# Happy-ZZX/PL-VIWO

Hardware: AMD Instinct MI355X
Metric: frames/sec (track+EKF update), 752x480 mono, 250 pts+80 lines; ATE vs CPU ref (higher is better)
Workload: dtype f64

## Files before the change

### pl-viwo_amd/csrc/dense_kernels.hip

```cpp
#include "mfma_tile.hpp"
#include "update_kernels.hpp"
#include "wave_ops.hpp"

namespace plv {


static inline int cdiv(int a, int b) { return (a + b - 1) / b; }

__global__ void __launch_bounds__(256) gram_direct_kernel(const double *__restrict__ A, int lda, int nc, const int *__restrict__ acc_rows, int F,
                                                          int mp_max, double *__restrict__ G, const int *__restrict__ skip,
                                                          double *__restrict__ Gs, double *__restrict__ gv) {
  if (skip && *skip == 0) return;
  __shared__ double part[3][256];
  const int nt = (nc + 15) >> 4;
  int rem = blockIdx.x, ti = 0;
  while (rem >= nt - ti) {
    rem -= nt - ti;
    ++ti;
  }
  const int tj = ti + rem;
  const int wave = threadIdx.x >> 6, lane = threadIdx.x & 63, li = lane & 15;
  const double *ai = A + (size_t)min(ti * 16 + li, nc - 1) * lda;
  const double *aj = A + (size_t)min(tj * 16 + li, nc - 1) * lda;
  d4 acc = {0, 0, 0, 0};
// ... 96 lines not shown
    for (int i = threadIdx.x; i < mirror2_words; i += blockDim.x) mirror2_dst[i] = mirror2_src[i];
  if (!(skipped || capped || *flag != 0)) {
    for (int idx = blockIdx.x * blockDim.x + threadIdx.x; idx < n * n; idx += gridDim.x * blockDim.x) {
      int j = idx / n, i = idx - j * n;
      if (i <= j) {
        const double u = P[(size_t)j * ldp + i];
        if (save) save[(size_t)j * n + i] = u, save[(size_t)i * n + j] = P[(size_t)i * ldp + j];
        double v = u - dC[(size_t)j * ldc + i];
        P[(size_t)j * ldp + i] = v;
        P[(size_t)i * ldp + j] = v;
      }
    }
  }
}

bool ekf_fast_fits(int r) { return r <= 192; }
static int launch_ekf_commit(plv_ctx *ctx, double *d_P, int n, int ldp, const double *dC, double *d_dx, int *d_flag, const void *mirror_src,
                             void *mirror_dst, size_t mirror_bytes);

int launch_ekf_fast(plv_ctx *ctx, double *d_P, int n, int ldp, const double *d_H, int r, int k, int ldh, const int *d_cols,
                    const double *d_res, const double *d_Rdiag, double *d_dx, int *d_flag, bool gathered, const void *mirror_src,
                    void *mirror_dst, size_t mirror_bytes) {
  int rc;
  const int ldm = r, ldw = r;
  if ((rc = ctx->d_Mt.reserve((size_t)r * (n + 1 + k) * 8)) || (rc = ctx->d_S.reserve((size_t)r * r * 8 * 2)) ||
      (rc = ctx->d_W.reserve((size_t)r * (n + 1) * 8)) || (rc = ctx->d_y.reserve((size_t)n * n * 8)))
    return rc;
  double *Mt = ctx->d_Mt.as<double>(), *S = ctx->d_S.as<double>(), *W = ctx->d_W.as<double>(), *dC = ctx->d_y.as<double>();
  launch_ekf_ms(ctx, d_P, n, ldp, d_H, r, k, ldh, d_cols, d_Rdiag, Mt, ldm, S, gathered, d_flag);
  if ((rc = launch_bchol_ekf(ctx, S, r, r, Mt, ldm, n, d_res, W, ldw, d_flag))) return rc;
  {
    ProfScope ps(ctx->prof, "ekf_dc_kernel", ctx->stream);
    int tn = cdiv(n + 1, 16);
    int waves = tn * (tn + 1) / 2;
    hipLaunchKernelGGL(ekf_dc_kernel, dim3(cdiv(waves, 4)), dim3(256), 0, ctx->stream, W, ldw, r, n, dC, n, d_dx, d_P, ldp, d_flag, ctx->skip_word,
                       (const double *)nullptr, (const double *)nullptr, (const double *)nullptr, (const int *)nullptr);
  }
  return launch_ekf_commit(ctx, d_P, n, ldp, dC, d_dx, d_flag, mirror_src, mirror_dst, mirror_bytes);
}

static int launch_ekf_commit(plv_ctx *ctx, double *d_P, int n, int ldp, const double *dC, double *d_dx, int *d_flag, const void *mirror_src,
                             void *mirror_dst, size_t mirror_bytes) {
  {
    ProfScope ps(ctx->prof, "ekf_commit_kernel", ctx->stream);
    hipLaunchKernelGGL(ekf_commit_kernel, dim3(std::min(64, cdiv(n * n, 256))), dim3(256), 0, ctx->stream, d_P, ldp, n, dC, n,
                       d_flag, (const unsigned *)mirror_src, (unsigned *)mirror_dst, (int)(mirror_bytes / 4), ctx->skip_word, d_dx,
                       (const unsigned *)(mirror_dst ? ctx->mirror2_src : nullptr), (unsigned *)(mirror_dst ? ctx->mirror2_dst : nullptr),
                       (int)((ctx->mirror2_bytes + 3) / 4), mirror_dst ? ctx->applied_word : nullptr,
                       mirror_dst ? ctx->cap_words : nullptr, ctx->cap, ctx->cov_save, ctx->cov_save_word, ctx->cov_save_seq);
    if (mirror_dst && ctx->applied_word) ctx->applied_used = true;
    if (mirror_dst && ctx->mirror2_dst) ctx->mirror2_taken = true;
  }
  PLV_HIP_CHECK(hipGetLastError());
// ... 113 lines not shown
                        void *mirror_dst, size_t mirror_bytes) {
  int rc;
  if ((rc = ctx->d_Mt.reserve((size_t)k * 8)) || (rc = ctx->d_S.reserve((size_t)k * k * 8)) || (rc = ctx->d_W.reserve((size_t)k * (n + 1) * 8)) ||
      (rc = ctx->d_y.reserve((size_t)n * n * 8)))
    return rc;
  double *cv = ctx->d_Mt.as<double>(), *B = ctx->d_S.as<double>(), *V = ctx->d_W.as<double>(), *dC = ctx->d_y.as<double>();
  const double *Gs = ctx->d_Gs.as<double>(), *gv = Gs + (size_t)k * k;
  if ((rc = ctx->d_C1.reserve(((size_t)n * n + n) * 8)) || (rc = ctx->d_Y0.reserve((size_t)k * (n + 1) * 8)) || (rc = ctx->d_GP.reserve((size_t)k * n * 8)))
    return rc;
  double *Y0 = ctx->d_Y0.as<double>(), *C1 = ctx->d_C1.as<double>(), *d0 = C1 + (size_t)n * n, *GP = ctx->d_GP.as<double>();
  const int *use_m = ctx->d_prior_near.as<int>();
  if (plv::knob(plv::PLV_KNOB_FORCE_FACTOR_FORM)) {
    static const int one[2] = {1, 0};
    PLV_HIP_CHECK(hipMemcpyAsync(ctx->d_prior_near.p, one, 8, hipMemcpyHostToDevice, ctx->stream));
  }
  launch_whiten_b(ctx, ctx->d_Lt.as<double>(), k, Gs, gv, cv, B, d_flag, d_P, ldp, n, d_cols, Y0, GP, d0, use_m);
  const WhitenC1Args wc{d_P, ldp, d_cols, GP, C1, Y0, use_m};
  if ((rc = launch_bchol_ekf(ctx, B, k, k, ctx->d_W0.as<double>(), k, n, cv, V, k, d_flag, &wc))) return rc;
  {
    ProfScope ps(ctx->prof, "ekf_dc_kernel", ctx->stream);
    const int tn = cdiv(n + 1, 16), waves = tn * (tn + 1) / 2;
    hipLaunchKernelGGL(ekf_dc_kernel, dim3(cdiv(waves, 4)), dim3(256), 0, ctx->stream, V, k, k, n, dC, n, d_dx, d_P, ldp, d_flag, ctx->skip_word,
                       ctx->d_dW.as<double>(), C1, d0, use_m);
  }
  return launch_ekf_commit(ctx, d_P, n, ldp, dC, d_dx, d_flag, mirror_src, mirror_dst, mirror_bytes);
}

}
```

### pl-viwo_amd/csrc/line_api.hip

```cpp
#include <algorithm>
#include <chrono>
#include <cmath>
#include <cstring>
#include <atomic>
#include <condition_variable>
#include <functional>
#include <memory>
#include <map>
#include <mutex>
#include <thread>
#include <unordered_map>
#include <vector>

#include "line_host.hpp"
#include "cam_models.hpp"
#include "line_kernels.hpp"
#include "update_state.hpp"
#include "plv_internal.hpp"
#include "camera_tracks.hpp"
#include "update_tail.hpp"

using namespace plv;
using namespace plv::linehost;

// ... 62 lines not shown
  struct WalkInfo {
    int mode = 0, n_components = 0, longest_component = 0, n_chains = 0, fell_back = 0;
  } winfo;
  bool chains_valid = false;
  std::vector<FldChain> last_chains;
  int last_pts_extent = 0;
  DevBuf comps, recs, recs_sorted;
  bool prefetch = false;
  std::unordered_map<uint64_t, LineTrack> db;
  DevBuf half, map, work, pts, chains, counts, segs, seg_count, uv_in, uv_out;
  DevBuf lab, lab_cnt, lab_roots;
  hipStream_t ccl_stream = nullptr;
  hipEvent_t canny_done = nullptr, labels_ready = nullptr;
  PinBuf pin;
  hipEvent_t edges_ready = nullptr;
  std::vector<uint64_t> dec_ids;
  std::vector<double> dec_vals;
  const uint8_t *early_raw = nullptr;
  const unsigned *early_hist = nullptr;
  int early_w = 0, early_h = 0;
  int pending_which = -1, pending_fed = -1;
  bool defer_finish = false;
  std::function<void()> deferred;
  std::atomic<int> defer_state{0};
  struct TriState {
    bool valid = false;
    plv_state_view view;
    std::vector<double> clone_time, clone_R, clone_p;
    std::vector<int> clone_id;
  } tri_state;
// ... 65 lines not shown
      F.pool_on = false;
      plv::frame_mark("@ (worker) line feed + pool done");
      plv::counters().w_feed_ns += (unsigned long long)std::chrono::duration_cast<std::chrono::nanoseconds>(std::chrono::steady_clock::now() - Fs).count();
      {
        std::lock_guard<std::mutex> lk(T->jm);
        F.rc = rc;
        T->feed_state = 2;
      }
      T->jcv.notify_all();
      continue;
    }
    const bool timing = plv::knob(plv::PLV_KNOB_LINE_TIMING);
    auto W0 = std::chrono::steady_clock::now();
    (void)hipSetDevice(T->job.device);
    int rc = PLV_OK;
    if (plv::event_sync(T->edges_ready) != hipSuccess) rc = PLV_E_DEVICE;
    if (rc == PLV_OK && T->job.hlab && plv::event_sync(T->labels_ready) != hipSuccess) rc = PLV_E_DEVICE;
    auto W1 = std::chrono::steady_clock::now();
    if (rc == PLV_OK) rc = host_extract(&T->host, T->job, timing);
    {
      auto ns = [](auto a, auto b) { return (unsigned long long)std::chrono::duration_cast<std::chrono::nanoseconds>(b - a).count(); };
      plv::counters().w_wake_ns += ns(T->job_posted, W0);
      plv::counters().w_maps_ns += ns(W0, W1);
      plv::counters().w_extract_ns += ns(W1, std::chrono::steady_clock::now());
    }
    if (plv::host_phases().on)
      plv::host_phases().add("line worker: detect job, post to done", std::chrono::duration<double, std::micro>(std::chrono::steady_clock::now() - T->job_posted).count());
    plv::frame_mark("@ (worker) line detection done");
    if (timing) {
      auto W2 = std::chrono::steady_clock::now();
      auto us = [](auto a, auto b) { return std::chrono::duration<double, std::micro>(b - a).count(); };
// ... 119 lines not shown
    b.lab_cnt = T->lab_cnt.as<int>();
    b.lab_roots = T->lab_roots.as<int>();
    b.comps = T->comps.as<FldComp>();
    b.recs = T->recs.as<FldRec>();
    b.recs_sorted = T->recs_sorted.as<FldRec>();
    b.walk_info = T->counts.as<int>() + 4;
  }
  if (!prelaunched) TRY(launch_line_edges(ctx, d_img, W, H, fp, b, ctx->stream, early ? T->early_hist : nullptr));
  if (with_labels && !T->ccl_stream) {
    PLV_HIP_CHECK(hipStreamCreateWithFlags(&T->ccl_stream, hipStreamNonBlocking));
    PLV_HIP_CHECK(hipEventCreateWithFlags(&T->canny_done, hipEventDisableTiming));
    PLV_HIP_CHECK(hipEventCreateWithFlags(&T->labels_ready, hipEventDisableTiming));
  }
  if (with_labels) PLV_HIP_CHECK(hipEventRecord(T->canny_done, ctx->stream));
  if (launch_only && !T->edges_ready) PLV_HIP_CHECK(hipEventCreateWithFlags(&T->edges_ready, hipEventDisableTiming));
  if (launch_only && maps_to_host) PLV_HIP_CHECK(hipEventRecord(T->edges_ready, ctx->stream));
  if (early && ctx->after_edges) TRY(ctx->after_edges(ctx->after_edges_arg));
  if (with_labels) {
    PLV_HIP_CHECK(hipStreamWaitEvent(T->ccl_stream, T->canny_done, 0));
    TRY(launch_line_labels(ctx, w, h, b, T->ccl_stream, fp.length_threshold));
    PLV_HIP_CHECK(hipEventRecord(T->labels_ready, T->ccl_stream));
  }
  const float thr2 = ctx->cfg.line_min_length_px * ctx->cfg.line_min_length_px;
  auto emit = [&](const float4 &sg) {
    const float x1 = sg.x * 2, y1 = sg.y * 2, x2 = sg.z * 2, y2 = sg.w * 2;
    const float l2 = (x2 - x1) * (x2 - x1) + (y2 - y1) * (y2 - y1);
    if (!(l2 > thr2)) return;
    lines.insert(lines.end(), {x1, y1, x2, y2});
  };
  lines.clear();
  if (!T->walk_on_device) {
// ... 1012 lines not shown
```

### pl-viwo_amd/csrc/plv_api.hip

```cpp
#include <algorithm>
#include <cstdarg>
#include <dlfcn.h>
#include <cmath>
#include <mutex>

#include "plv_ctx.hpp"
#include "update_kernels.hpp"
#include "update_state.hpp"

namespace plv {

static thread_local char g_err[512] = "";
void set_last_error(const char *fmt, ...) {
  va_list ap;
  va_start(ap, fmt);
  vsnprintf(g_err, sizeof(g_err), fmt, ap);
  va_end(ap);
}

double chi2_quantile(int dof, double p);

Roctx::Roctx() {
  if (!getenv("PLV_ROCTX")) return;
  for (const char *name : {"librocprofiler-sdk-roctx.so", "libroctx64.so"}) {
// ... 225 lines not shown
    g_states.push_back({ctx, us});
  }
  *out = ctx;
  return PLV_OK;
}

void plv_ctx_destroy(plv_ctx *ctx) {
  if (!ctx) return;
  (void)hipSetDevice(ctx->device);
  (void)plv::stream_sync(ctx->stream);
  plv_tracker_destroy(ctx);
  plv_line_tracker_destroy(ctx);
  plv_frontend_destroy(ctx);
  ctx->prof.destroy();
  plv::DevBuf *bufs[] = {&ctx->d_P, &ctx->d_P2, &ctx->d_H, &ctx->d_res, &ctx->d_cols, &ctx->d_Rdiag, &ctx->d_dx, &ctx->d_flag,
                         &ctx->d_Mt, &ctx->d_S, &ctx->d_W, &ctx->d_y, &ctx->d_fHf, &ctx->d_fHx, &ctx->d_fres,
                         &ctx->d_frows, &ctx->d_chi2, &ctx->d_acc, &ctx->d_stack, &ctx->d_stack_l, &ctx->d_stack2, &ctx->d_Pc, &ctx->d_Ps,
                         &ctx->d_inv, &ctx->d_T, &ctx->d_Lt, &ctx->d_W0, &ctx->d_dW, &ctx->d_Gs};
  for (auto *b : bufs) b->release();
  if (ctx->aux_stream) {
    (void)plv::stream_sync(ctx->aux_stream);
    (void)hipStreamDestroy(ctx->aux_stream);
  }
  if (ctx->aux_fork) (void)hipEventDestroy(ctx->aux_fork);
  if (ctx->aux_join) (void)hipEventDestroy(ctx->aux_join);
  ctx->h_pin.release();
  ctx->h_pin_flow.release();
  ctx->h_pin_l.release();
  plv_ctx_update_state *us = nullptr;
  {
    std::lock_guard<std::mutex> lk(g_state_mtx);
// ... 520 lines not shown
  const size_t rb = result_rows_off(n, F) + (size_t)F * 4;
  plv::PinBuf &hpin = ctx->res_pin(fdim);
  TRY(hpin.reserve(rb));
  struct SkipGuard {
    plv_ctx *c;
    ~SkipGuard() { c->skip_word = nullptr; }
  } skip_guard{ctx};
  const bool whiten = whitened_route(us, Mtot, k);
  bool aux_open = prior_was_pending;
  auto aux_join = [&]() -> int {
    if (!aux_open) return PLV_OK;
    aux_open = false;
    PLV_HIP_CHECK(hipStreamWaitEvent(ctx->stream, ctx->aux_join, 0));
    return PLV_OK;
  };
  const bool probing = ctx->probe && !us->graph_mode;
  auto start_prior = [&]() -> int {
    TRY(aux_join());
    TRY(prior_mark(ctx, true));
    TRY(prior_start(ctx, us->bcols_of(fdim).as<int>(), k));
    aux_open = true;
    return PLV_OK;
  };
  auto enqueue = [&]() -> int {
  if (whiten && !prefetched && !probing) TRY(start_prior());
  if (!projected) {
    TRY(launch_nullspace(ctx, F, fdim, k, ld, us->brows.as<int>(), wHf, wHx, wres, ctx->d_P.as<double>(), n, n, us->bcols_of(fdim).as<int>()));
  } else if (!gathers_valid) {
    TRY(launch_gather_cov(ctx, ctx->d_P.as<double>(), n, n, us->bcols_of(fdim).as<int>(), k));
  }
  Chi2Args a{};
// ... 19 lines not shown
    ctx->dec_F_l = F;
  }
  a.stack = ctx->stack_of(fdim).as<double>();
  a.lds = Mtot;
  a.mp_max = mp_max;
  a.chi2_mult = chi2_mult;
  a.res_norm_gate = res_norm_gate;
  a.q95 = us->q95.as<double>();
  a.q95_n = Q95_N;
  a.min_rows = fdim == 3 ? 4 : 5;
  a.accepted = d_acc;
  a.acc_rows = d_acc_rows;
  a.n_acc = d_flag + 1;
  a.stack_accepted_only = (Mtot > k && k <= 192 && whiten) ? 1 : 0;
  ctx->skip_word = (Mtot > k ? k <= 192 : ekf_fast_fits(Mtot)) ? d_flag + 1 : nullptr;
  const bool probe = ctx->probe && !us->graph_mode;
  if (probe) {
    char *hb = hpin.as<char>();
    a.h_accepted = (unsigned char *)(hb + (size_t)n * 8 + 16);
    a.h_acc_rows = (int *)(hb + result_rows_off(n, F));
    a.probe_src = (const unsigned char *)ctx->probe_src;
    a.probe_dst = (unsigned char *)ctx->probe_dst;
    a.probe_stride_a = ctx->probe_stride_a, a.probe_off_b = ctx->probe_off_b, a.probe_stride_b = ctx->probe_stride_b;
  }
  const bool gated = ctx->gate_stage_taken && projected && ctx->gate_stage.stack == a.stack && ctx->gate_stage.lds == a.lds &&
                     ctx->gate_stage.accepted == a.accepted && ctx->gate_stage.stack_accepted_only == a.stack_accepted_only;
  if (ctx->gate_stage_taken && !gated) {
    set_last_error("plv_msckf_update_resident: the batch was gated inside its Jacobian launch for other buffers than this update's");
    return PLV_E_BADARG;
  }
  if (gated) {
// ... 11 lines not shown
    if (ctx->probe_hook) ctx->probe_hook(ctx->probe_hook_arg);
    TRY(sync(ctx));
    const unsigned char *hacc = (const unsigned char *)(hpin.as<char>() + (size_t)n * 8 + 16);
    int any = 0;
    for (int f = 0; f < F; ++f) any |= hacc[f];
    if (!any) {
      memset(hpin.p, 0, (size_t)n * 8 + 16);
      ctx->probe_done = true;
      return aux_join();
    }
    const int *hrows = (const int *)(hpin.as<char>() + result_rows_off(n, F));
    int m_acc = 0;
    for (int f = 0; f < F; ++f) m_acc += std::max(hrows[f], 0);
    if (whiten && m_acc > 0 && m_acc <= k && ekf_fast_fits(m_acc) && !plv::knob(plv::PLV_KNOB_FORCE_FACTOR_FORM)) {
      TRY(ctx->d_stackc.reserve((size_t)m_acc * nc * 8));
      TRY(launch_stack_compact(ctx, ctx->stack_of(fdim).as<double>(), Mtot, nc, d_acc_rows, F, mp_max, ctx->d_stackc.as<double>(), m_acc, true));
      TRY(aux_join());
      const double *Hc = ctx->d_stackc.as<double>();
      TRY(launch_ekf_fast(ctx, ctx->d_P.as<double>(), n, n, Hc, m_acc, k, m_acc, us->bcols_of(fdim).as<int>(), Hc + (size_t)k * m_acc, nullptr, d_dx, d_flag,
                          gathers_valid, resbuf.p, hpin.p, (rb + 3) & ~(size_t)3));
      us->last_route = 0;
      return PLV_OK;
    }
    if (whiten && !prefetched) TRY(start_prior());
  }

  const double *dH, *dr;
  int r, ldh;
  if (whiten) {
    TRY(launch_gram_information(ctx, ctx->stack_of(fdim).as<double>(), Mtot, nc, d_acc_rows, F, mp_max));
// ... 219 lines not shown
```

### pl-viwo_amd/csrc/plv_ctx.hpp

```cpp
#pragma once
#include <hip/hip_runtime.h>
#include <sys/resource.h>

#include "gate_stage.hpp"
#include <cstdint>
#include <cstdio>
#include <execinfo.h>
#include <cstring>
#include <algorithm>
#include <atomic>
#include <chrono>
#include <cstdlib>
#include <mutex>
#include <string>
#include <unordered_map>
#include <vector>

#include "../../include/plviwo.h"

namespace plv {

void set_last_error(const char *fmt, ...);

#define PLV_HIP_CHECK(expr)                                                              \
// ... 33 lines not shown
  counters().copy_bytes += bytes;
  return hipMemcpyAsync(dst, src, bytes, kind, s);
}

enum : unsigned { PLV_KNOB_PRIOR_LATE = 2u, PLV_KNOB_GATE_SEPARATE = 1024u, PLV_KNOB_NO_CHAIN = 2048u, PLV_KNOB_CHAIN_ALWAYS = 4096u,
                  PLV_KNOB_FORCE_FACTOR_FORM = 8192u,
                  PLV_KNOB_HOST_TIMING = 1u << 14,
                  PLV_KNOB_LINE_TIMING = 1u << 15,
                  PLV_KNOB_UPDATE_TIMING = 1u << 16,
                  PLV_KNOB_KERNEL_STAMPS = 1u << 17,
                  PLV_KNOB_CHAIN_EVENTS = 1u << 18,
                  PLV_KNOB_ALLOC_DEBUG = 1u << 19,
                  PLV_KNOB_HOST_FAULTS = 1u << 20,
                  PLV_KNOB_NO_SPECULATION = 1u << 24,
                  PLV_KNOB_HELPER_NAPS = 1u << 28,
                  PLV_KNOB_TSQR_TREE = 1u << 29 };
inline std::atomic<unsigned> &knobs() {
  static std::atomic<unsigned> k{getenv("PLV_DEBUG_KNOBS") ? (unsigned)strtoul(getenv("PLV_DEBUG_KNOBS"), nullptr, 0) : 0u};
  return k;
}
inline bool knob(unsigned bit) { return (knobs().load(std::memory_order_relaxed) & bit) != 0; }
inline bool alloc_debug() { return knob(PLV_KNOB_ALLOC_DEBUG); }

struct HostPhases {
  struct Rec {
    const char *label;
    double us = 0;
    long n = 0;
    float last[64] = {};
    void put(double v) {
      last[n & 63] = (float)v;
// ... 302 lines not shown

struct plv_ctx {
  plv_config cfg;
  int cam_model = 0;
  int device = 0;
  hipStream_t stream = nullptr;
  plv::Profiler prof;

  int cov_n = 0;
  unsigned long long gather_stamp = 1;
  unsigned long long cov_host_synced = 0;
  plv::DevBuf d_P;
  plv::DevBuf d_P2;
  plv::DevBuf d_H, d_res, d_cols, d_Rdiag, d_dx, d_flag;
  plv::DevBuf d_Mt, d_S, d_W, d_y;
  plv::DevBuf d_Pc, d_Ps, d_inv, d_T;
  plv::DevBuf d_fHf, d_fHx, d_fres, d_frows, d_chi2, d_acc;
  void (*edges_hook)(plv_ctx *, const uint8_t *d_raw, int W, int H, const unsigned *d_hist) = nullptr;
  bool edges_hook_fired = false;
  int (*after_edges)(void *) = nullptr;
  void *after_edges_arg = nullptr;
  bool decision_trace = false;
  plv::DevBuf d_tri_dbg, d_gate_dec, d_gate_dec_l;
  int dec_F_l = 0;
  int dec_F = 0;
  bool dec_gate = false;
  plv::DevBuf d_stack, d_stack2;
  plv::DevBuf d_stack_l;
  plv::DevBuf &stack_of(int fdim) { return fdim == 6 ? d_stack_l : d_stack; }
  plv::DevBuf d_Lt, d_W0, d_dW, d_Gs, d_GP, d_Y0, d_C1, d_stackc;
// ... 49 lines not shown
```

### pl-viwo_amd/csrc/update_kernels.hip

```cpp
#include <algorithm>

#include "plv_ctx.hpp"
#include "blocked_chol.hpp"
#include "mfma_tile.hpp"
#include "nullspace_core.hpp"
#include "update_kernels.hpp"

namespace plv {

template <class FA, class FB>
__device__ __forceinline__ d4 mfma_tile_f64(FA a, FB b, int K, d4 acc) {
  const int lane = threadIdx.x & 63;
  const int ij = lane & 15, kq = lane >> 4;
  int k0 = 0;
  for (; k0 + 16 <= K; k0 += 16) {
    double av[4], bv[4];
#pragma unroll
    for (int u = 0; u < 4; ++u) {
      av[u] = a(ij, k0 + 4 * u + kq);
      bv[u] = b(k0 + 4 * u + kq, ij);
    }
#pragma unroll
    for (int u = 0; u < 4; ++u) acc = __builtin_amdgcn_mfma_f64_16x16x4f64(av[u], bv[u], acc, 0, 0, 0);
  }
// ... 576 lines not shown
  const double *P;
  int ldp, n;
  const int *cols;
  const double *g;
  double *Y0;
  double *GP;
  double *d0;
  const int *use_m;
  int first;
};

__global__ void __launch_bounds__(512) ekf_ms_kernel(const double *__restrict__ H, int ldh, int r, int k, const double *__restrict__ Pc,
                                                     int ldp, int n, const double *__restrict__ Ps, double *__restrict__ Mt, int ldm,
                                                     const double *__restrict__ Rdiag, double *__restrict__ S, int lds_,
                                                     int mt_blocks, int *__restrict__ flag, const int *__restrict__ skip, int h_upper,
                                                     WhitenPanels wp) {
  __shared__ double strip[192 * 17];
  if (flag && blockIdx.x == 0 && threadIdx.x == 0) {
    flag[0] = 0;
  }
  if (skip && *skip == 0) return;
  const int wave = threadIdx.x >> 6, lane = threadIdx.x & 63, li = lane & 15, nw = blockDim.x >> 6;
  if ((int)blockIdx.x < mt_blocks) {
    const int tr_n = (r + 15) >> 4, tn_n = (n + 15) >> 4;
    const int tile = blockIdx.x * nw + wave;
    if (tile >= tr_n * tn_n) return;
    const int tr = tile / tn_n, tn = tile - tr * tn_n;
    d4 acc = {0, 0, 0, 0};
    const int k0 = h_upper ? min(tr * 16, k) : 0;
    const double *Hr = H + min(tr * 16 + li, r - 1) + (size_t)k0 * ldh;
    const double *Pq = Pc + min(tn * 16 + li, n - 1) + (size_t)k0 * ldp;
    auto fa = [&](int, int kk) { return Hr[(size_t)kk * ldh]; };
    auto fb = [&](int kk, int) { return Pq[(size_t)kk * ldp]; };
    acc = mfma_tile_f64_pipe<16>(fa, fb, k - k0, acc);
#pragma unroll
    for (int q = 0; q < 4; ++q) {
      const int i = tr * 16 + (lane >> 4) + 4 * q, j = tn * 16 + li;
      if (i < r && j < n) Mt[(size_t)j * ldm + i] = acc[q];
    }
    return;
  }
  const int kt = (k + 15) >> 4, tr_n = (r + 15) >> 4;
  if (wp.first >= 0 && (int)blockIdx.x >= wp.first) {
    __shared__ int scols[192];
    if ((wp.use_m[0] | wp.use_m[1]) == 0) return;
// ... 28 lines not shown
      const double *sp = strip + k0 * 17;
      auto fa = [&](int, int kk) { return Hr[(size_t)kk * ldh]; };
      auto fb = [&](int kk, int) { return sp[kk * 17 + li]; };
      acc = mfma_tile_f64_pipe<16>(fa, fb, k - k0, acc);
#pragma unroll
      for (int q = 0; q < 4; ++q) {
        const int c = tj * 16 + (lane >> 4) + 4 * q;
        if (c < k && b0 + li < wp.n) wp.Y0[(size_t)(b0 + li) * k + c] = acc[q];
      }
    }
    return;
  }
  const int ti = blockIdx.x - mt_blocks;
  {
    const int k0 = h_upper ? min(ti * 16, k) : 0;
    const double *Hr = H + min(ti * 16 + li, r - 1) + (size_t)k0 * ldh;
    for (int tj = wave; tj < kt; tj += nw) {
      d4 acc = {0, 0, 0, 0};
      const double *Pq = Ps + min(tj * 16 + li, k - 1) + (size_t)k0 * k;
      auto fa = [&](int, int kk) { return Hr[(size_t)kk * ldh]; };
      auto fb = [&](int kk, int) { return Pq[(size_t)kk * k]; };
      acc = mfma_tile_f64_pipe<16>(fa, fb, k - k0, acc);
#pragma unroll
      for (int q = 0; q < 4; ++q) {
        const int j = tj * 16 + li;
        if (j < k) strip[j * 17 + (lane >> 4) + 4 * q] = acc[q];
      }
    }
  }
  __syncthreads();
  for (int tj = ti + wave; tj < tr_n; tj += nw) {
    d4 acc = {0, 0, 0, 0};
    const int k0 = h_upper ? min(tj * 16, k) : 0;
    const double *Hc = H + min(tj * 16 + li, r - 1) + (size_t)k0 * ldh;
    const double *sp = strip + k0 * 17;
    auto fa = [&](int, int kk) { return sp[kk * 17 + li]; };
    auto fb = [&](int kk, int) { return Hc[(size_t)kk * ldh]; };
    acc = mfma_tile_f64_pipe<16>(fa, fb, k - k0, acc);
#pragma unroll
    for (int q = 0; q < 4; ++q) {
      const int i = ti * 16 + (lane >> 4) + 4 * q, j = tj * 16 + li;
      if (i < r && j < r) S[(size_t)j * lds_ + i] = acc[q] + (i == j ? (Rdiag ? Rdiag[i] : 1.0) : 0.0);
    }
  }
}

__global__ void __launch_bounds__(1024) ekf_chol_kernel(const double *__restrict__ S, int lds_, int r, double *__restrict__ L,
                                                        int ldl, int *__restrict__ flag) {
  extern __shared__ double smem[];
// ... 242 lines not shown
      *result = dst;
      *ld_out = ldo;
      return PLV_OK;
    }
    rows = W * nc;
    src_ld = ldo;
    double *t = src;
    src = dst;
    dst = t;
    size_t tc = cap_src;
    cap_src = cap_dst;
    cap_dst = tc;
  }
}

void launch_ekf_ms(plv_ctx *ctx, const double *d_P, int n, int ldp, const double *d_H, int r, int k, int ldh,
                   const int *d_cols, const double *d_Rdiag, double *Mt, int ldm, double *S, bool gathered, int *d_flag) {
  if (!gathered) (void)launch_gather_cov(ctx, d_P, n, ldp, d_cols, k);
  ProfScope ps(ctx->prof, "ekf_ms_kernel", ctx->stream);
  const int mt_blocks = cdiv(cdiv(r, 16) * cdiv(n, 16), 4);
  if (k > 192) {
    hipLaunchKernelGGL(ekf_mt_kernel, dim3(mt_blocks), dim3(256), 0, ctx->stream, d_H, ldh, r, k, ctx->d_inv.as<int>(),
                       ctx->d_Pc.as<double>(), n, n, Mt, ldm, d_flag, ctx->skip_word);
    hipLaunchKernelGGL(ekf_s_kernel, dim3(cdiv(cdiv(r, 16) * cdiv(r, 16), 4)), dim3(256), 0, ctx->stream, Mt + (size_t)(n + 1) * ldm, ldm,
                       d_H, ldh, r, k, d_cols, d_Rdiag, S, r, ctx->skip_word);
    return;
  }
  hipLaunchKernelGGL(ekf_ms_kernel, dim3(mt_blocks + cdiv(r, 16)), dim3(256), 0, ctx->stream, d_H, ldh, r, k, ctx->d_Pc.as<double>(), n, n,
                     ctx->d_Ps.as<double>(), Mt, ldm, d_Rdiag, S, r, mt_blocks, d_flag, ctx->skip_word, 0, WhitenPanels{nullptr, 0, 0, nullptr, nullptr, nullptr, nullptr, nullptr, nullptr, -1});
}

void launch_whiten_b(plv_ctx *ctx, const double *Lt, int k, const double *Gs, const double *gv, double *cv, double *B, int *d_flag,
                     const double *d_P, int ldp, int n, const int *d_cols, double *Y0, double *GP, double *d0, const int *use_m) {
  ProfScope ps(ctx->prof, "ekf_ms_kernel", ctx->stream);
  const int mt_blocks = cdiv(cdiv(k, 16), 8), first = mt_blocks + cdiv(k, 16);
  hipLaunchKernelGGL(ekf_ms_kernel, dim3(first + cdiv(n, 16)), dim3(512), 0, ctx->stream, Lt, k, k, k, gv, 1, 1, Gs, cv, k,
                     (const double *)nullptr, B, k, mt_blocks, d_flag, ctx->skip_word, 1, WhitenPanels{d_P, ldp, n, d_cols, gv, Y0, GP, d0, use_m, first});
}

int launch_ekf(plv_ctx *ctx, double *d_P, int n, int ldp, const double *d_H, int r, int k, int ldh, const int *d_cols,
               const double *d_res, const double *d_Rdiag, double *d_dx, int *d_flag, bool gathered) {
  int rc;
  const int ldm = r, ldw = r;
  if ((rc = ctx->d_Mt.reserve((size_t)r * (n + 1 + k) * 8)) || (rc = ctx->d_S.reserve((size_t)r * r * 8 * 2)) ||
      (rc = ctx->d_W.reserve((size_t)r * (n + 1) * 8)))
    return rc;
  double *Mt = ctx->d_Mt.as<double>(), *S = ctx->d_S.as<double>(), *L = S + (size_t)r * r, *W = ctx->d_W.as<double>();
  size_t shm = (size_t)r * (r | 1) * sizeof(double);
  if (shm > 160 * 1024) {
    set_last_error("ekf: r=%d exceeds the LDS-resident Cholesky capacity", r);
    return PLV_E_CAPACITY;
  }
// ... 25 lines not shown
```

### pl-viwo_amd/csrc/update_kernels.hpp

```cpp
#pragma once
#include "plv_ctx.hpp"

namespace plv {

struct Chi2Args {
  const double *P;
  int ldp;
  int k, ld, fdim_off;
  const int *rows;
  const double *Hx, *res;
  const int *cols;
  double sigma2;
  double *chi2;
  double *dec;
  double *stack;
  int lds, mp_max;
  double chi2_mult, res_norm_gate;
  const double *q95;
  int q95_n;
  int min_rows;
  unsigned char *accepted;
  int *acc_rows;
  int *n_acc;
  int stack_accepted_only;
// ... 7 lines not shown
  int probe_stride_a, probe_off_b, probe_stride_b;
};

int launch_nullspace(plv_ctx *ctx, int F, int fdim, int k, int ld, const int *d_rows, double *d_Hf, double *d_Hx,
                     double *d_res, const double *d_P = nullptr, int n = 0, int ldp = 0, const int *d_cols = nullptr,
                     int shift = -1 );
struct GatherArgs;
int gather_args(plv_ctx *ctx, const double *d_P, int n, int ldp, const int *d_cols, int k, GatherArgs &g);
int launch_gather_cov(plv_ctx *ctx, const double *d_P, int n, int ldp, const int *d_cols, int k);
int launch_chi2(plv_ctx *ctx, int F, const Chi2Args &a, int max_mp);
int launch_tsqr(plv_ctx *ctx, double *d_A, int lda, int m, int nc, double *d_tmp, size_t tmp_elems, double **result,
                int *ld_out, const int *m_dev = nullptr);
int launch_ekf(plv_ctx *ctx, double *d_P, int n, int ldp, const double *d_H, int r, int k, int ldh, const int *d_cols,
               const double *d_res, const double *d_Rdiag, double *d_dx, int *d_flag, bool gathered = false);

void launch_ekf_ms(plv_ctx *ctx, const double *d_P, int n, int ldp, const double *d_H, int r, int k, int ldh,
                   const int *d_cols, const double *d_Rdiag, double *Mt, int ldm, double *S, bool gathered = false,
                   int *d_flag = nullptr);
bool ekf_fast_fits(int r);
int launch_ekf_fast(plv_ctx *ctx, double *d_P, int n, int ldp, const double *d_H, int r, int k, int ldh, const int *d_cols,
                    const double *d_res, const double *d_Rdiag, double *d_dx, int *d_flag, bool gathered = false, const void *mirror_src = nullptr,
                    void *mirror_dst = nullptr, size_t mirror_bytes = 0);

void launch_whiten_b(plv_ctx *ctx, const double *Lt, int k, const double *Gs, const double *gv, double *cv, double *B, int *d_flag,
                     const double *d_P, int ldp, int n, const int *d_cols, double *Y0, double *GP, double *d0, const int *use_m);
int launch_stack_compact(plv_ctx *ctx, const double *d_A, int lda, int nc, const int *d_acc_rows, int F, int mp_max, double *d_dst, int ldd, bool exact_rows = false,
                         int *d_total_out = nullptr );
int launch_cov_restore(plv_ctx *ctx, double *d_P, int n, const double *save, const unsigned *save_word, unsigned seq);
int launch_stack_zero_rejected(plv_ctx *ctx, double *d_A, int lda, int nc, const int *d_acc_rows, int F, int mp_max);
int launch_prior_factor(plv_ctx *ctx, hipStream_t st, const double *d_P, int n, int ldp, const int *d_cols, int k);
int launch_gram_information(plv_ctx *ctx, const double *d_A, int lda, int nc, const int *d_acc_rows, int F, int mp_max);
int launch_ekf_whitened(plv_ctx *ctx, double *d_P, int n, int ldp, int k, const int *d_cols, double *d_dx, int *d_flag, const void *mirror_src, void *mirror_dst,
                        size_t mirror_bytes);
int launch_bchol_prior(plv_ctx *ctx, hipStream_t st, const double *d_P, int ldp, int n, const int *d_cols, int k, double *d_Lt, int ldl,
                       double *d_W0, int ldw, int *d_n_near);

int launch_cov_init_invertible(plv_ctx *ctx, const double *d_P, int n, const int *d_cols, int k, const double *d_Hx, const double *d_Hf,
                               const double *d_res, int ld, double *d_Pn, double *d_out, int *d_flag);

struct WhitenC1Args {
// ... 13 lines not shown
```

Measured before the change: 2001.

## Fuse EKF covariance-delta and commit into one kernel, read accepted rows in place

Adds a single-launch ekf_dc_commit kernel. Each block computes a tile of the covariance downdate and checks the diagonal for negativity using P's diagonal, which the ms kernel snapshots. It also writes dx, the mirror copies and P in place, replacing the separate dc and commit kernels and the dC scratch round-trip. The ms kernel can now read accepted measurement rows through a row map, so the stack-compaction launch is skipped on the whitened fast path. Line extraction waits on the canny event instead of a separate edges event. Together these cut launch count and memory traffic on the update tail, at the cost of a much more complex kernel and more blocks being launched.

```diff
diff --git a/pl-viwo_amd/csrc/dense_kernels.hip b/pl-viwo_amd/csrc/dense_kernels.hip
--- a/pl-viwo_amd/csrc/dense_kernels.hip
+++ b/pl-viwo_amd/csrc/dense_kernels.hip
@@ -134,29 +134,180 @@
   }
 }
 
+template <int NW, int CH>
+__global__ void __launch_bounds__(64 * NW) ekf_dc_commit_kernel(const double *__restrict__ W, int ldw, int r, int n, double *__restrict__ dx,
+                                                            double *__restrict__ P, int ldp, const double *__restrict__ pdiag,
+                                                            int *__restrict__ flag, const int *__restrict__ skip,
+                                                            const double *__restrict__ dW, const double *__restrict__ C1,
+                                                            const double *__restrict__ d0, const int *__restrict__ use_m,
+                                                            const unsigned *__restrict__ mirror_src, unsigned *__restrict__ mirror_dst,
+                                                            int mirror_words, int dx_word, int flag_word,
+                                                            const unsigned *__restrict__ mirror2_src, unsigned *__restrict__ mirror2_dst,
+                                                            int mirror2_words, int *__restrict__ applied_out,
+                                                            const int *__restrict__ cap_words, int cap, double *__restrict__ save,
+                                                            unsigned *__restrict__ save_word, unsigned save_seq) {
+  __shared__ int s_neg[16];
+  const bool skipped = skip && *skip == 0;
+  const bool capped = cap_words && cap_words[0] != 0 && cap_words[1] >= cap;
+  const int before = *flag;
+  const int tn = (n + 1 + 15) >> 4;
+  const int wave = threadIdx.x >> 6, lane = threadIdx.x & 63, li = lane & 15;
+  if (mirror2_dst && blockIdx.x == gridDim.x - 1)
+    for (int i = threadIdx.x; i < mirror2_words; i += blockDim.x) mirror2_dst[i] = mirror2_src[i];
+  if (skipped) {
+    if (blockIdx.x != 0) return;
+    const int status = before | (capped ? 16 : 0);
+    if (threadIdx.x == 0) {
+      if (capped) atomicOr(flag, 16);
+      if (applied_out) *applied_out = 0;
+      if (save_word) *save_word = 0u;
+    }
+    if (dx)
+      for (int i = threadIdx.x; i < n; i += blockDim.x) dx[i] = 0.0;
+    if (mirror_dst)
+      for (int i = threadIdx.x; i < mirror_words; i += blockDim.x)
+        mirror_dst[i] = i == flag_word ? (unsigned)status : (dx_word >= 0 && i >= dx_word && i < dx_word + 2 * n) ? 0u : mirror_src[i];
+    return;
+  }
+  const bool fm = use_m && (use_m[0] | use_m[1]) != 0;
+  if (fm) dW = C1;
+  int ti = 0, rem = blockIdx.x;
+  while (rem >= tn - ti) {
+    rem -= tn - ti;
+    ++ti;
+  }
+  int tj = ti + rem;
+  const bool own = wave == tn;
+  if (!own) ti = tj = wave;
+  if (mirror_dst && blockIdx.x == 0)
+    for (int i = threadIdx.x; i < mirror_words; i += blockDim.x)
+      if (i != flag_word && !(dx_word >= 0 && i >= dx_word && i < dx_word + 2 * n)) mirror_dst[i] = mirror_src[i];
+  double dwv[4], pu[4], pl[4], pdv = 0.0;
+#pragma unroll
+  for (int q = 0; q < 4; ++q) {
+    const int i = ti * 16 + (lane >> 4) + 4 * q, j = tj * 16 + li, ic = min(i, n - 1), jc = min(j, n - 1);
+    dwv[q] = dW ? dW[(size_t)jc * n + ic] : 0.0;
+    if (!own && i == j) pdv = pdiag[ic];
+    pu[q] = own ? P[(size_t)jc * ldp + ic] : 0.0;
+    pl[q] = own && save ? P[(size_t)ic * ldp + jc] : 0.0;
+  }
+  const double *Wi = W + (size_t)min(ti * 16 + li, n) * ldw;
+  const double *Wj = W + (size_t)min(tj * 16 + li, n) * ldw;
+  d4 acc = {0, 0, 0, 0};
+  auto fa = [&](int, int kk) { return Wi[kk]; };
+  if (own) {
+    auto fb = [&](int kk, int) { return Wj[kk]; };
+    acc = mfma_tile_f64_pipe<CH>(fa, fb, r, acc);
+  } else {
+    auto fb = [&](int kk, int) { return Wi[kk]; };
+    acc = mfma_tile_f64_pipe<CH>(fa, fb, r, acc);
+  }
+  double v[4];
+  bool bad = false;
+#pragma unroll
+  for (int q = 0; q < 4; ++q) {
+    const int i = ti * 16 + (lane >> 4) + 4 * q, j = tj * 16 + li;
+    v[q] = (dW && i < n && j < n) ? dwv[q] - acc[q] : acc[q];
+    if (!own && i == j && i < n && pdv - v[q] < 0.0) bad = true;
+    if (own && dx && i < n && j == n) {
+      const double d = fm ? d0[i] - acc[q] : acc[q];
+      dx[i] = d;
+      if (mirror_dst && dx_word >= 0) ((double *)(mirror_dst + dx_word))[i] = d;
+    }
+  }
+  if (!own) {
+    const unsigned long long any = __ballot(bad);
+    if (lane == 0) s_neg[wave] = any != 0ull ? 1 : 0;
+  }
+  __syncthreads();
+  int neg = 0;
+  for (int d = 0; d < tn; ++d) neg |= s_neg[d];
+  const int status = before | neg | (capped ? 16 : 0);
+  if (blockIdx.x == 0 && threadIdx.x == 0) {
+    if (status != before) atomicOr(flag, status);
+    if (applied_out) *applied_out = status != 0 ? 0 : 1;
+    if (save_word) *save_word = status != 0 ? 0u : save_seq;
+    if (mirror_dst && flag_word >= 0) mirror_dst[flag_word] = (unsigned)status;
+  }
+  if (status != 0 || !own) return;
+#pragma unroll
+  for (int q = 0; q < 4; ++q) {
+    const int i = ti * 16 + (lane >> 4) + 4 * q, j = tj * 16 + li;
+    if (i <= j && j < n) {
+      if (save) save[(size_t)j * n + i] = pu[q], save[(size_t)i * n + j] = pl[q];
+      const double w = pu[q] - v[q];
+      P[(size_t)j * ldp + i] = w;
+      P[(size_t)i * ldp + j] = w;
+    }
+  }
+}
+
 bool ekf_fast_fits(int r) { return r <= 192; }
 static int launch_ekf_commit(plv_ctx *ctx, double *d_P, int n, int ldp, const double *dC, double *d_dx, int *d_flag, const void *mirror_src,
                              void *mirror_dst, size_t mirror_bytes);
+static bool ekf_tail_one_launch(int tn);
+static int launch_ekf_dc_commit(plv_ctx *ctx, const double *W, int ldw, int r, int n, double *d_dx, double *d_P, int ldp, const double *pdiag, int *d_flag,
+                                const double *dW, const double *C1, const double *d0, const int *use_m, const void *mirror_src, void *mirror_dst,
+                                size_t mirror_bytes);
 
 int launch_ekf_fast(plv_ctx *ctx, double *d_P, int n, int ldp, const double *d_H, int r, int k, int ldh, const int *d_cols,
                     const double *d_res, const double *d_Rdiag, double *d_dx, int *d_flag, bool gathered, const void *mirror_src,
-                    void *mirror_dst, size_t mirror_bytes) {
+                    void *mirror_dst, size_t mirror_bytes, const EkfRowMap *rm) {
   int rc;
+  if (rm && k > 192) {
+    set_last_error("launch_ekf_fast: rows in place with %d columns", k);
+    return PLV_E_CAPACITY;
+  }
   const int ldm = r, ldw = r;
   if ((rc = ctx->d_Mt.reserve((size_t)r * (n + 1 + k) * 8)) || (rc = ctx->d_S.reserve((size_t)r * r * 8 * 2)) ||
       (rc = ctx->d_W.reserve((size_t)r * (n + 1) * 8)) || (rc = ctx->d_y.reserve((size_t)n * n * 8)))
     return rc;
   double *Mt = ctx->d_Mt.as<double>(), *S = ctx->d_S.as<double>(), *W = ctx->d_W.as<double>(), *dC = ctx->d_y.as<double>();
-  launch_ekf_ms(ctx, d_P, n, ldp, d_H, r, k, ldh, d_cols, d_Rdiag, Mt, ldm, S, gathered, d_flag);
-  if ((rc = launch_bchol_ekf(ctx, S, r, r, Mt, ldm, n, d_res, W, ldw, d_flag))) return rc;
+  const int tn = cdiv(n + 1, 16);
+  const bool one = ekf_tail_one_launch(tn);
+  double *pdiag = nullptr;
+  if (one) {
+    if ((rc = ctx->d_pdiag.reserve((size_t)n * 8))) return rc;
+    pdiag = ctx->d_pdiag.as<double>();
+  }
+  const bool filled = launch_ekf_ms(ctx, d_P, n, ldp, d_H, r, k, ldh, d_cols, d_Rdiag, Mt, ldm, S, gathered, d_flag, pdiag, rm);
+  if ((rc = launch_bchol_ekf(ctx, S, r, r, Mt, ldm, n, rm ? rm->res_out : d_res, W, ldw, d_flag))) return rc;
+  if (one && filled)
+    return launch_ekf_dc_commit(ctx, W, ldw, r, n, d_dx, d_P, ldp, pdiag, d_flag, nullptr, nullptr, nullptr, nullptr, mirror_src, mirror_dst, mirror_bytes);
   {
     ProfScope ps(ctx->prof, "ekf_dc_kernel", ctx->stream);
-    int tn = cdiv(n + 1, 16);
     int waves = tn * (tn + 1) / 2;
     hipLaunchKernelGGL(ekf_dc_kernel, dim3(cdiv(waves, 4)), dim3(256), 0, ctx->stream, W, ldw, r, n, dC, n, d_dx, d_P, ldp, d_flag, ctx->skip_word,
                        (const double *)nullptr, (const double *)nullptr, (const double *)nullptr, (const int *)nullptr);
   }
   return launch_ekf_commit(ctx, d_P, n, ldp, dC, d_dx, d_flag, mirror_src, mirror_dst, mirror_bytes);
+}
+
+static bool ekf_tail_one_launch(int tn) { return tn + 1 <= 16 && !plv::knob(plv::PLV_KNOB_UPDATE_TAIL_OLD); }
+static int launch_ekf_dc_commit(plv_ctx *ctx, const double *W, int ldw, int r, int n, double *d_dx, double *d_P, int ldp, const double *pdiag, int *d_flag,
+                                const double *dW, const double *C1, const double *d0, const int *use_m, const void *mirror_src, void *mirror_dst,
+                                size_t mirror_bytes) {
+  const int tn = cdiv(n + 1, 16), words = (int)(mirror_bytes / 4);
+  auto word_of = [&](const void *p, size_t bytes) -> int {
+    if (!mirror_dst || !p) return -1;
+    const ptrdiff_t off = (const char *)p - (const char *)mirror_src;
+    return off >= 0 && off % 8 == 0 && (size_t)off + bytes <= mirror_bytes ? (int)(off / 4) : -1;
+  };
+  const int dx_word = word_of(d_dx, (size_t)n * 8), flag_word = word_of(d_flag, 4);
+  {
+    ProfScope ps(ctx->prof, "ekf_dc_commit_kernel", ctx->stream);
+    auto *kern = ekf_dc_commit_kernel<12, 12>;
+    if (tn + 1 > 12) kern = ekf_dc_commit_kernel<16, 8>;
+    hipLaunchKernelGGL(kern, dim3(tn * (tn + 1) / 2), dim3(64 * (tn + 1)), 0, ctx->stream, W, ldw, r, n, d_dx, d_P, ldp, pdiag, d_flag,
+                       ctx->skip_word, dW, C1, d0, use_m, (const unsigned *)mirror_src, (unsigned *)mirror_dst, words, dx_word, flag_word,
+                       (const unsigned *)(mirror_dst ? ctx->mirror2_src : nullptr), (unsigned *)(mirror_dst ? ctx->mirror2_dst : nullptr),
+                       (int)((ctx->mirror2_bytes + 3) / 4), mirror_dst ? ctx->applied_word : nullptr, mirror_dst ? ctx->cap_words : nullptr, ctx->cap,
+                       ctx->cov_save, ctx->cov_save_word, ctx->cov_save_seq);
+    if (mirror_dst && ctx->applied_word) ctx->applied_used = true;
+    if (mirror_dst && ctx->mirror2_dst) ctx->mirror2_taken = true;
+  }
+  PLV_HIP_CHECK(hipGetLastError());
+  return PLV_OK;
 }
 
 static int launch_ekf_commit(plv_ctx *ctx, double *d_P, int n, int ldp, const double *dC, double *d_dx, int *d_flag, const void *mirror_src,
@@ -300,12 +451,21 @@
     static const int one[2] = {1, 0};
     PLV_HIP_CHECK(hipMemcpyAsync(ctx->d_prior_near.p, one, 8, hipMemcpyHostToDevice, ctx->stream));
   }
-  launch_whiten_b(ctx, ctx->d_Lt.as<double>(), k, Gs, gv, cv, B, d_flag, d_P, ldp, n, d_cols, Y0, GP, d0, use_m);
+  const int tn = cdiv(n + 1, 16);
+  const bool one = ekf_tail_one_launch(tn);
+  double *pdiag = nullptr;
+  if (one) {
+    if ((rc = ctx->d_pdiag.reserve((size_t)n * 8))) return rc;
+    pdiag = ctx->d_pdiag.as<double>();
+  }
+  launch_whiten_b(ctx, ctx->d_Lt.as<double>(), k, Gs, gv, cv, B, d_flag, d_P, ldp, n, d_cols, Y0, GP, d0, use_m, pdiag);
   const WhitenC1Args wc{d_P, ldp, d_cols, GP, C1, Y0, use_m};
   if ((rc = launch_bchol_ekf(ctx, B, k, k, ctx->d_W0.as<double>(), k, n, cv, V, k, d_flag, &wc))) return rc;
+  if (one)
+    return launch_ekf_dc_commit(ctx, V, k, k, n, d_dx, d_P, ldp, pdiag, d_flag, ctx->d_dW.as<double>(), C1, d0, use_m, mirror_src, mirror_dst, mirror_bytes);
   {
     ProfScope ps(ctx->prof, "ekf_dc_kernel", ctx->stream);
-    const int tn = cdiv(n + 1, 16), waves = tn * (tn + 1) / 2;
+    const int waves = tn * (tn + 1) / 2;
     hipLaunchKernelGGL(ekf_dc_kernel, dim3(cdiv(waves, 4)), dim3(256), 0, ctx->stream, V, k, k, n, dC, n, d_dx, d_P, ldp, d_flag, ctx->skip_word,
                        ctx->d_dW.as<double>(), C1, d0, use_m);
   }
diff --git a/pl-viwo_amd/csrc/line_api.hip b/pl-viwo_amd/csrc/line_api.hip
--- a/pl-viwo_amd/csrc/line_api.hip
+++ b/pl-viwo_amd/csrc/line_api.hip
@@ -100,6 +100,7 @@
   hipEvent_t canny_done = nullptr, labels_ready = nullptr;
   PinBuf pin;
   hipEvent_t edges_ready = nullptr;
+  hipEvent_t maps_event = nullptr;
   std::vector<uint64_t> dec_ids;
   std::vector<double> dec_vals;
   const uint8_t *early_raw = nullptr;
@@ -195,7 +196,7 @@
     auto W0 = std::chrono::steady_clock::now();
     (void)hipSetDevice(T->job.device);
     int rc = PLV_OK;
-    if (plv::event_sync(T->edges_ready) != hipSuccess) rc = PLV_E_DEVICE;
+    if (plv::event_sync(T->maps_event) != hipSuccess) rc = PLV_E_DEVICE;
     if (rc == PLV_OK && T->job.hlab && plv::event_sync(T->labels_ready) != hipSuccess) rc = PLV_E_DEVICE;
     auto W1 = std::chrono::steady_clock::now();
     if (rc == PLV_OK) rc = host_extract(&T->host, T->job, timing);
@@ -345,7 +346,9 @@
   }
   if (with_labels) PLV_HIP_CHECK(hipEventRecord(T->canny_done, ctx->stream));
   if (launch_only && !T->edges_ready) PLV_HIP_CHECK(hipEventCreateWithFlags(&T->edges_ready, hipEventDisableTiming));
-  if (launch_only && maps_to_host) PLV_HIP_CHECK(hipEventRecord(T->edges_ready, ctx->stream));
+  const bool maps_on_canny = with_labels && maps_to_host && !plv::knob(plv::PLV_KNOB_UPDATE_TAIL_OLD);
+  if (launch_only && maps_to_host && !maps_on_canny) PLV_HIP_CHECK(hipEventRecord(T->edges_ready, ctx->stream));
+  if (launch_only) T->maps_event = maps_on_canny ? T->canny_done : T->edges_ready;
   if (early && ctx->after_edges) TRY(ctx->after_edges(ctx->after_edges_arg));
   if (with_labels) {
     PLV_HIP_CHECK(hipStreamWaitEvent(T->ccl_stream, T->canny_done, 0));
diff --git a/pl-viwo_amd/csrc/plv_api.hip b/pl-viwo_amd/csrc/plv_api.hip
--- a/pl-viwo_amd/csrc/plv_api.hip
+++ b/pl-viwo_amd/csrc/plv_api.hip
@@ -263,7 +263,7 @@
   plv_frontend_destroy(ctx);
   ctx->prof.destroy();
   plv::DevBuf *bufs[] = {&ctx->d_P, &ctx->d_P2, &ctx->d_H, &ctx->d_res, &ctx->d_cols, &ctx->d_Rdiag, &ctx->d_dx, &ctx->d_flag,
-                         &ctx->d_Mt, &ctx->d_S, &ctx->d_W, &ctx->d_y, &ctx->d_fHf, &ctx->d_fHx, &ctx->d_fres,
+                         &ctx->d_Mt, &ctx->d_S, &ctx->d_W, &ctx->d_y, &ctx->d_pdiag, &ctx->d_fHf, &ctx->d_fHx, &ctx->d_fres,
                          &ctx->d_frows, &ctx->d_chi2, &ctx->d_acc, &ctx->d_stack, &ctx->d_stack_l, &ctx->d_stack2, &ctx->d_Pc, &ctx->d_Ps,
                          &ctx->d_inv, &ctx->d_T, &ctx->d_Lt, &ctx->d_W0, &ctx->d_dW, &ctx->d_Gs};
   for (auto *b : bufs) b->release();
@@ -814,7 +814,7 @@
     PLV_HIP_CHECK(hipStreamWaitEvent(ctx->stream, ctx->aux_join, 0));
     return PLV_OK;
   };
-  const bool probing = ctx->probe && !us->graph_mode;
+  const bool probing = (ctx->probe || plv::knob(plv::PLV_KNOB_PROBE_ALWAYS)) && !us->graph_mode;
   auto start_prior = [&]() -> int {
     TRY(aux_join());
     TRY(prior_mark(ctx, true));
@@ -864,7 +864,7 @@
   a.n_acc = d_flag + 1;
   a.stack_accepted_only = (Mtot > k && k <= 192 && whiten) ? 1 : 0;
   ctx->skip_word = (Mtot > k ? k <= 192 : ekf_fast_fits(Mtot)) ? d_flag + 1 : nullptr;
-  const bool probe = ctx->probe && !us->graph_mode;
+  const bool probe = probing;
   if (probe) {
     char *hb = hpin.as<char>();
     a.h_accepted = (unsigned char *)(hb + (size_t)n * 8 + 16);
@@ -906,6 +906,14 @@
     for (int f = 0; f < F; ++f) m_acc += std::max(hrows[f], 0);
     if (whiten && m_acc > 0 && m_acc <= k && ekf_fast_fits(m_acc) && !plv::knob(plv::PLV_KNOB_FORCE_FACTOR_FORM)) {
       TRY(ctx->d_stackc.reserve((size_t)m_acc * nc * 8));
+      if (k <= 192 && !plv::knob(plv::PLV_KNOB_UPDATE_TAIL_OLD)) {
+        TRY(aux_join());
+        const plv::EkfRowMap rm{d_acc_rows, F, mp_max, ctx->d_stackc.as<double>()};
+        TRY(launch_ekf_fast(ctx, ctx->d_P.as<double>(), n, n, ctx->stack_of(fdim).as<double>(), m_acc, k, Mtot, us->bcols_of(fdim).as<int>(), nullptr, nullptr,
+                            d_dx, d_flag, gathers_valid, resbuf.p, hpin.p, (rb + 3) & ~(size_t)3, &rm));
+        us->last_route = 0;
+        return PLV_OK;
+      }
       TRY(launch_stack_compact(ctx, ctx->stack_of(fdim).as<double>(), Mtot, nc, d_acc_rows, F, mp_max, ctx->d_stackc.as<double>(), m_acc, true));
       TRY(aux_join());
       const double *Hc = ctx->d_stackc.as<double>();
diff --git a/pl-viwo_amd/csrc/plv_ctx.hpp b/pl-viwo_amd/csrc/plv_ctx.hpp
--- a/pl-viwo_amd/csrc/plv_ctx.hpp
+++ b/pl-viwo_amd/csrc/plv_ctx.hpp
@@ -71,7 +71,9 @@
                   PLV_KNOB_HOST_FAULTS = 1u << 20,
                   PLV_KNOB_NO_SPECULATION = 1u << 24,
                   PLV_KNOB_HELPER_NAPS = 1u << 28,
-                  PLV_KNOB_TSQR_TREE = 1u << 29 };
+                  PLV_KNOB_TSQR_TREE = 1u << 29,
+                  PLV_KNOB_UPDATE_TAIL_OLD = 1u << 30,
+                  PLV_KNOB_PROBE_ALWAYS = 1u << 31 };
 inline std::atomic<unsigned> &knobs() {
   static std::atomic<unsigned> k{getenv("PLV_DEBUG_KNOBS") ? (unsigned)strtoul(getenv("PLV_DEBUG_KNOBS"), nullptr, 0) : 0u};
   return k;
@@ -404,6 +406,7 @@
   plv::DevBuf d_P2;
   plv::DevBuf d_H, d_res, d_cols, d_Rdiag, d_dx, d_flag;
   plv::DevBuf d_Mt, d_S, d_W, d_y;
+  plv::DevBuf d_pdiag;
   plv::DevBuf d_Pc, d_Ps, d_inv, d_T;
   plv::DevBuf d_fHf, d_fHx, d_fres, d_frows, d_chi2, d_acc;
   void (*edges_hook)(plv_ctx *, const uint8_t *d_raw, int W, int H, const unsigned *d_hist) = nullptr;
diff --git a/pl-viwo_amd/csrc/update_kernels.hip b/pl-viwo_amd/csrc/update_kernels.hip
--- a/pl-viwo_amd/csrc/update_kernels.hip
+++ b/pl-viwo_amd/csrc/update_kernels.hip
@@ -614,13 +614,41 @@
                                                      int ldp, int n, const double *__restrict__ Ps, double *__restrict__ Mt, int ldm,
                                                      const double *__restrict__ Rdiag, double *__restrict__ S, int lds_,
                                                      int mt_blocks, int *__restrict__ flag, const int *__restrict__ skip, int h_upper,
-                                                     WhitenPanels wp) {
+                                                     WhitenPanels wp, double *__restrict__ pdiag, const double *__restrict__ pd_P, int pd_ldp,
+                                                     int pd_n, EkfRowMap rm) {
   __shared__ double strip[192 * 17];
   if (flag && blockIdx.x == 0 && threadIdx.x == 0) {
     flag[0] = 0;
   }
   if (skip && *skip == 0) return;
+  if (pdiag && blockIdx.x == 0)
+    for (int i = threadIdx.x; i < pd_n; i += blockDim.x) pdiag[i] = pd_P[(size_t)i * pd_ldp + i];
   const int wave = threadIdx.x >> 6, lane = threadIdx.x & 63, li = lane & 15, nw = blockDim.x >> 6;
+  __shared__ int srow[192];
+  if (rm.acc_rows) {
+    if (wave == 0) {
+      int base = 0;
+      for (int f0 = 0; f0 < rm.F; f0 += 64) {
+        const int f = f0 + lane;
+        const int rows = f < rm.F ? min(max(rm.acc_rows[f], 0), rm.mp_max) : 0;
+        int incl = rows;
+#pragma unroll
+        for (int o = 1; o < 64; o <<= 1) {
+          const int t = __shfl_up(incl, o, 64);
+          if (lane >= o) incl += t;
+        }
+        const int off = base + incl - rows;
+        for (int i = 0; i < rows; ++i)
+          if (off + i < 192) srow[off + i] = f * rm.mp_max + i;
+        base += __shfl(incl, 63, 64);
+      }
+      for (int i = base + lane; i < 192; i += 64) srow[i] = 0;
+    }
+    __syncthreads();
+    if (blockIdx.x == 0 && rm.res_out)
+      for (int i = threadIdx.x; i < r; i += blockDim.x) rm.res_out[i] = H[(size_t)k * ldh + srow[i]];
+  }
+  auto hrow = [&](int i) { return rm.acc_rows ? srow[i] : i; };
   if ((int)blockIdx.x < mt_blocks) {
     const int tr_n = (r + 15) >> 4, tn_n = (n + 15) >> 4;
     const int tile = blockIdx.x * nw + wave;
@@ -628,7 +656,7 @@
     const int tr = tile / tn_n, tn = tile - tr * tn_n;
     d4 acc = {0, 0, 0, 0};
     const int k0 = h_upper ? min(tr * 16, k) : 0;
-    const double *Hr = H + min(tr * 16 + li, r - 1) + (size_t)k0 * ldh;
+    const double *Hr = H + hrow(min(tr * 16 + li, r - 1)) + (size_t)k0 * ldh;
     const double *Pq = Pc + min(tn * 16 + li, n - 1) + (size_t)k0 * ldp;
     auto fa = [&](int, int kk) { return Hr[(size_t)kk * ldh]; };
     auto fb = [&](int kk, int) { return Pq[(size_t)kk * ldp]; };
@@ -687,7 +715,7 @@
   const int ti = blockIdx.x - mt_blocks;
   {
     const int k0 = h_upper ? min(ti * 16, k) : 0;
-    const double *Hr = H + min(ti * 16 + li, r - 1) + (size_t)k0 * ldh;
+    const double *Hr = H + hrow(min(ti * 16 + li, r - 1)) + (size_t)k0 * ldh;
     for (int tj = wave; tj < kt; tj += nw) {
       d4 acc = {0, 0, 0, 0};
       const double *Pq = Ps + min(tj * 16 + li, k - 1) + (size_t)k0 * k;
@@ -705,7 +733,7 @@
   for (int tj = ti + wave; tj < tr_n; tj += nw) {
     d4 acc = {0, 0, 0, 0};
     const int k0 = h_upper ? min(tj * 16, k) : 0;
-    const double *Hc = H + min(tj * 16 + li, r - 1) + (size_t)k0 * ldh;
+    const double *Hc = H + hrow(min(tj * 16 + li, r - 1)) + (size_t)k0 * ldh;
     const double *sp = strip + k0 * 17;
     auto fa = [&](int, int kk) { return sp[kk * 17 + li]; };
     auto fb = [&](int kk, int) { return Hc[(size_t)kk * ldh]; };
@@ -978,8 +1006,9 @@
   }
 }
 
-void launch_ekf_ms(plv_ctx *ctx, const double *d_P, int n, int ldp, const double *d_H, int r, int k, int ldh,
-                   const int *d_cols, const double *d_Rdiag, double *Mt, int ldm, double *S, bool gathered, int *d_flag) {
+bool launch_ekf_ms(plv_ctx *ctx, const double *d_P, int n, int ldp, const double *d_H, int r, int k, int ldh,
+                   const int *d_cols, const double *d_Rdiag, double *Mt, int ldm, double *S, bool gathered, int *d_flag, double *pdiag,
+                   const EkfRowMap *rm) {
   if (!gathered) (void)launch_gather_cov(ctx, d_P, n, ldp, d_cols, k);
   ProfScope ps(ctx->prof, "ekf_ms_kernel", ctx->stream);
   const int mt_blocks = cdiv(cdiv(r, 16) * cdiv(n, 16), 4);
@@ -988,18 +1017,21 @@
                        ctx->d_Pc.as<double>(), n, n, Mt, ldm, d_flag, ctx->skip_word);
     hipLaunchKernelGGL(ekf_s_kernel, dim3(cdiv(cdiv(r, 16) * cdiv(r, 16), 4)), dim3(256), 0, ctx->stream, Mt + (size_t)(n + 1) * ldm, ldm,
                        d_H, ldh, r, k, d_cols, d_Rdiag, S, r, ctx->skip_word);
-    return;
+    return false;
   }
   hipLaunchKernelGGL(ekf_ms_kernel, dim3(mt_blocks + cdiv(r, 16)), dim3(256), 0, ctx->stream, d_H, ldh, r, k, ctx->d_Pc.as<double>(), n, n,
-                     ctx->d_Ps.as<double>(), Mt, ldm, d_Rdiag, S, r, mt_blocks, d_flag, ctx->skip_word, 0, WhitenPanels{nullptr, 0, 0, nullptr, nullptr, nullptr, nullptr, nullptr, nullptr, -1});
+                     ctx->d_Ps.as<double>(), Mt, ldm, d_Rdiag, S, r, mt_blocks, d_flag, ctx->skip_word, 0, WhitenPanels{nullptr, 0, 0, nullptr, nullptr, nullptr, nullptr, nullptr, nullptr, -1},
+                     pdiag, d_P, ldp, n, rm ? *rm : EkfRowMap{nullptr, 0, 0, nullptr});
+  return pdiag != nullptr;
 }
 
 void launch_whiten_b(plv_ctx *ctx, const double *Lt, int k, const double *Gs, const double *gv, double *cv, double *B, int *d_flag,
-                     const double *d_P, int ldp, int n, const int *d_cols, double *Y0, double *GP, double *d0, const int *use_m) {
+                     const double *d_P, int ldp, int n, const int *d_cols, double *Y0, double *GP, double *d0, const int *use_m, double *pdiag) {
   ProfScope ps(ctx->prof, "ekf_ms_kernel", ctx->stream);
   const int mt_blocks = cdiv(cdiv(k, 16), 8), first = mt_blocks + cdiv(k, 16);
   hipLaunchKernelGGL(ekf_ms_kernel, dim3(first + cdiv(n, 16)), dim3(512), 0, ctx->stream, Lt, k, k, k, gv, 1, 1, Gs, cv, k,
-                     (const double *)nullptr, B, k, mt_blocks, d_flag, ctx->skip_word, 1, WhitenPanels{d_P, ldp, n, d_cols, gv, Y0, GP, d0, use_m, first});
+                     (const double *)nullptr, B, k, mt_blocks, d_flag, ctx->skip_word, 1, WhitenPanels{d_P, ldp, n, d_cols, gv, Y0, GP, d0, use_m, first}, pdiag, d_P, ldp, n,
+                     EkfRowMap{nullptr, 0, 0, nullptr});
 }
 
 int launch_ekf(plv_ctx *ctx, double *d_P, int n, int ldp, const double *d_H, int r, int k, int ldh, const int *d_cols,
diff --git a/pl-viwo_amd/csrc/update_kernels.hpp b/pl-viwo_amd/csrc/update_kernels.hpp
--- a/pl-viwo_amd/csrc/update_kernels.hpp
+++ b/pl-viwo_amd/csrc/update_kernels.hpp
@@ -45,16 +45,22 @@
 int launch_ekf(plv_ctx *ctx, double *d_P, int n, int ldp, const double *d_H, int r, int k, int ldh, const int *d_cols,
                const double *d_res, const double *d_Rdiag, double *d_dx, int *d_flag, bool gathered = false);
 
-void launch_ekf_ms(plv_ctx *ctx, const double *d_P, int n, int ldp, const double *d_H, int r, int k, int ldh,
+struct EkfRowMap {
+  const int *acc_rows;
+  int F, mp_max;
+  double *res_out;
+};
+bool launch_ekf_ms(plv_ctx *ctx, const double *d_P, int n, int ldp, const double *d_H, int r, int k, int ldh,
                    const int *d_cols, const double *d_Rdiag, double *Mt, int ldm, double *S, bool gathered = false,
-                   int *d_flag = nullptr);
+                   int *d_flag = nullptr, double *pdiag = nullptr, const EkfRowMap *rm = nullptr);
 bool ekf_fast_fits(int r);
 int launch_ekf_fast(plv_ctx *ctx, double *d_P, int n, int ldp, const double *d_H, int r, int k, int ldh, const int *d_cols,
                     const double *d_res, const double *d_Rdiag, double *d_dx, int *d_flag, bool gathered = false, const void *mirror_src = nullptr,
-                    void *mirror_dst = nullptr, size_t mirror_bytes = 0);
+                    void *mirror_dst = nullptr, size_t mirror_bytes = 0, const EkfRowMap *rm = nullptr );
 
 void launch_whiten_b(plv_ctx *ctx, const double *Lt, int k, const double *Gs, const double *gv, double *cv, double *B, int *d_flag,
-                     const double *d_P, int ldp, int n, const int *d_cols, double *Y0, double *GP, double *d0, const int *use_m);
+                     const double *d_P, int ldp, int n, const int *d_cols, double *Y0, double *GP, double *d0, const int *use_m,
+                     double *pdiag = nullptr);
 int launch_stack_compact(plv_ctx *ctx, const double *d_A, int lda, int nc, const int *d_acc_rows, int F, int mp_max, double *d_dst, int ldd, bool exact_rows = false,
                          int *d_total_out = nullptr );
 int launch_cov_restore(plv_ctx *ctx, double *d_P, int n, const double *save, const unsigned *save_word, unsigned seq);
```

After: 1946. 2.8% lower.
